# decadenza/SimpleStereo

Measured on AMD Instinct MI355X. Metric: disparity MPixels/s (H*W*nDisp per second), higher is better.
Workload: dtype f32

## Files before the change

simplestereo_amd/csrc/asw_exact_kernels.hip.h:

```cpp
#pragma once
#include "asw_shared.hip.h"
#include "lab_kernels.hip.h"
#include "glibc_math.hip.h"

namespace ssamd {

struct AswExactArgs {
    const PixRec *recL, *recR;
    const double *labL, *labR;
    const double *prox;
    u64 *keyL, *keyR;
    int16_t *disp;
    AswExactQueue q;
    AswExactQueue raw;
    double *ecost;
    u64 *costL, *costR;
    uint32_t *idxL, *idxR;
    uint32_t *wslotL, *wslotR;
    uint32_t *wpix;
    double *wtab;
    unsigned int wcap;
    int H, W, win, pad, minD, maxD, row0, rows;
    double gammaC;
};

__device__ __forceinline__ double exact_sqrt(double x)
{
#pragma clang fp contract(off)
    const double y0 = sqrt(x);
    if (!(y0 > 0.0) || !(y0 < 1.0e300)) return y0;
    const double e = fma(-y0, y0, x);
    return y0 + e / (2.0 * y0);
}

__global__ __launch_bounds__(256) void bgr2lab_f64_pair_kernel(const PixRec *__restrict__ recL, const PixRec *__restrict__ recR,
                                                               double *__restrict__ labL, double *__restrict__ labR, long long npix)
{
    SSAMD_LAB_TABLES_IN_LDS(T)
    long long q = (long long)blockIdx.x * blockDim.x + threadIdx.x;
    const long long stride = (long long)gridDim.x * blockDim.x;
    for (; q < 2 * npix; q += stride) {
        const bool right = q >= npix;
        const long long p = right ? q - npix : q;
        const uint32_t v = (right ? recR : recL)[p].bgrx;
        double L, a, b;
        bgr_to_lab_f64(v & 0xff, (v >> 8) & 0xff, (v >> 16) & 0xff, L, a, b, T);
        double *const o = (right ? labR : labL) + 3 * p;
        o[0] = L; o[1] = a; o[2] = b;
    }
}

__device__ __forceinline__ bool exact_overflowed(const AswExactArgs &A)
{
    return A.q.counter[0] > A.q.cap || (A.raw.entries && A.raw.counter[0] > A.raw.cap);
}

__global__ __launch_bounds__(256) void asw_exact_filter_kernel(const AswExactArgs A)
{
    const unsigned n = min(A.raw.counter[0], A.raw.cap);
    const unsigned nloop = (n + 255u) & ~255u;
    for (unsigned e0 = blockIdx.x * blockDim.x; e0 < nloop; e0 += gridDim.x * blockDim.x) {
        const unsigned e = e0 + threadIdx.x;
        unsigned s2 = 0;
        uint32_t pix = 0, rkey = 0xffffffffu;
        int d = 0;
        if (e < n) {
            const u64 ent = A.raw.entries[e];
            const uint32_t key = A.raw.ekeys[e];
            rkey = key;
            pix = (uint32_t)ent;
            d = (int)((ent >> 32) & 0xffff);
            const unsigned sides = (unsigned)(ent >> 48) & 3u;
            const uint32_t esc = 0xC0000000u - __float_as_uint(2.0f * A.q.sat_abs);
            if (sides & EXACT_SIDE_L) {
                const u64 g = A.keyL[pix];
                if ((int)(uint32_t)g != d && (uint32_t)(g >> 32) < esc && exact_near(key, (uint32_t)(g >> 32), A.q.tol, A.q.sat_abs, exact_zkey(A.win))) s2 |= EXACT_SIDE_L;
            }
            if ((sides & EXACT_SIDE_R) && A.keyR) {
                const u64 g = A.keyR[pix - (uint32_t)d];
                if ((uint32_t)g != pix % (uint32_t)A.W && (uint32_t)(g >> 32) < esc && exact_near(key, (uint32_t)(g >> 32), A.q.tol, A.q.sat_abs, exact_zkey(A.win))) s2 |= EXACT_SIDE_R;
            }
        }
        asw_exact_push_wave(A.q, s2 != 0, pix, d, s2, rkey);
    }
}

__global__ __launch_bounds__(256) void asw_exact_escalate_kernel(const AswExactArgs A)
{
    const AswExactQueue &Q = A.q;
    const uint32_t esc = 0xC0000000u - __float_as_uint(2.0f * Q.sat_abs);
    const long long n = (long long)A.rows * A.W;
    for (long long q = (long long)blockIdx.x * blockDim.x + threadIdx.x; q < n; q += (long long)gridDim.x * blockDim.x) {
        const int x = (int)(q % A.W);
        const u64 gl = A.keyL[q];
        if (gl != KEY_NONE && (uint32_t)(gl >> 32) >= esc) {
            const int dwin = (int)(uint32_t)gl, dhi = min(A.maxD, x);
            const int cnt = dhi - A.minD;
            if (cnt > 0) {
                unsigned slot = atomicAdd(Q.counter, (unsigned)cnt);
                for (int d = A.minD; d <= dhi; ++d)
                    if (d != dwin) {
                        if (slot < Q.cap) Q.entries[slot] = exact_entry((uint32_t)q, d, EXACT_SIDE_L);
                        ++slot;
                    }
                Q.flagL[q] = 1;
            }
        }
        if (A.keyR) {
            const u64 gr = A.keyR[q];
            if (gr != KEY_NONE && (uint32_t)(gr >> 32) >= esc) {
                const int xwin = (int)(uint32_t)gr;
                const int dhi = min(A.maxD, A.W - 1 - x), cnt = dhi - A.minD;
                if (cnt > 0) {
                    unsigned slot = atomicAdd(Q.counter, (unsigned)cnt);
                    for (int d = A.minD; d <= dhi; ++d)
                        if (x + d != xwin) {
                            if (slot < Q.cap) Q.entries[slot] = exact_entry((uint32_t)(q + d), d, EXACT_SIDE_R);
                            ++slot;
                        }
                    Q.flagR[q] = 1;
                }
            }
        }
    }
}

static constexpr int EXACT_ZSEG = 64, EXACT_ZWIN_MAX = 64;
__global__ __launch_bounds__(256) void asw_exact_zero_kernel(const AswExactArgs A)
{
    extern __shared__ __attribute__((aligned(16))) char zsmem[];
    const AswExactQueue &Q = A.q;
// ... 32 lines not shown
            }
            if (__syncthreads_or(tid < EXACT_ZSEG && s_state[tid] == 1) == 0) continue;
            if (win >= EXACT_ZWIN_MAX) {
                if (tid < EXACT_ZSEG && s_state[tid] == 1) s_state[tid] = 3;
            } else {
                const PixRec *const imgA = side ? A.recR : A.recL, *const imgB = side ? A.recL : A.recR;
                auto stage = [&](uint32_t *tile, const PixRec *img, int shift) {
                    for (int k0 = 0; k0 < win * TW; k0 += 8 * 256) {
                        uint32_t v[8];
#pragma unroll
                        for (int u = 0; u < 8; ++u) {
                            const int k = k0 + u * 256 + tid, i = k / TW, c = k - i * TW, ii = y - p + i, cc = x0 - p + c + shift;
                            v[u] = (k < win * TW && (unsigned)ii < (unsigned)H && (unsigned)cc < (unsigned)W) ? img[(size_t)ii * W + cc].bgrx : 0x80000000u;
                        }
#pragma unroll
                        for (int u = 0; u < 8; ++u) {
                            const int k = k0 + u * 256 + tid;
                            if (k < win * TW) tile[k] = v[u];
                        }
                    }
                };
                stage(tA, imgA, 0);
                for (;;) {
                    __syncthreads();
                    if (tid == 0) {
                        int cur = -1;
                        for (int k = 0; k < EXACT_ZSEG; ++k)
                            if (s_state[k] == 1) { cur = side ? s_idx[k] - (x0 + k) : s_idx[k]; break; }
                        s_cur = cur;
                    }
                    __syncthreads();
                    const int d = s_cur;
                    if (d < 0) break;
                    const int shift = side ? d : -d;
                    stage(tB, imgB, shift);
                    __syncthreads();
                    const int px = tid & (EXACT_ZSEG - 1), part = tid >> 6;
                    const bool mine = s_state[px] == 1 && (side ? s_idx[px] - (x0 + px) : s_idx[px]) == d;
                    bool nz = false;
                    if (mine) {
                        uint32_t acc = 0;
                        for (int i = part; i < win; i += 4) {
                            const uint32_t *const ra = tA + i * TW + px, *const rb = tB + i * TW + px;
#pragma unroll 8
                            for (int j = 0; j < win; ++j) {
                                const uint32_t a = ra[j], b = rb[j];
                                acc |= ((a | b) >> 31) ? 0u : (a ^ b);
                            }
                        }
                        nz = acc != 0u;
                    }
                    __syncthreads();
                    if (mine && part == 0) s_state[px] = 2;
                    __syncthreads();
                    if (mine && nz) s_state[px] = 3;
                }
            }
            __syncthreads();
            if (tid < EXACT_ZSEG && s_state[tid] == 3) {
                const int xq = x0 + tid, widx = s_idx[tid];
                const long long pq = (long long)yr * W + xq;
                if (side == 0) {
                    const int dhi = min(A.maxD, xq), cnt = dhi - A.minD;
                    if (cnt > 0) {
                        unsigned slot = atomicAdd(Q.counter, (unsigned)cnt);
                        for (int d = A.minD; d <= dhi; ++d)
                            if (d != widx) { if (slot < Q.cap) Q.entries[slot] = exact_entry((uint32_t)pq, d, EXACT_SIDE_L); ++slot; }
                        Q.flagL[pq] = 1;
                    }
                } else {
                    const int dhi = min(A.maxD, W - 1 - xq), cnt = dhi - A.minD;
                    if (cnt > 0) {
                        unsigned slot = atomicAdd(Q.counter, (unsigned)cnt);
                        for (int d = A.minD; d <= dhi; ++d)
                            if (xq + d != widx) { if (slot < Q.cap) Q.entries[slot] = exact_entry((uint32_t)(pq + d), d, EXACT_SIDE_R); ++slot; }
                        Q.flagR[pq] = 1;
                    }
                }
            }
        }
    }
}

__device__ __forceinline__ void exact_assign_wslot(const AswExactArgs &A, bool flagged, u64 mask, uint32_t pix, uint32_t side)
{
    if (mask == 0 || A.wcap == 0) return;
    const int leader = (int)__builtin_ctzll(mask);
    const unsigned lane = __builtin_amdgcn_mbcnt_hi(~0u, __builtin_amdgcn_mbcnt_lo(~0u, 0u));
    unsigned base = 0;
    if ((int)lane == leader) base = atomicAdd(A.q.counter + 6, (unsigned)__builtin_popcountll(mask));
    base = (unsigned)__builtin_amdgcn_readlane((int)base, leader);
    if (flagged) {
        const unsigned slot = base + (unsigned)__builtin_popcountll(mask & (((u64)1 << lane) - 1));
        (side ? A.wslotR : A.wslotL)[pix] = slot;
        if (slot < A.wcap) A.wpix[slot] = pix | (side << 31);
    }
}

__global__ __launch_bounds__(256) void asw_exact_winners_kernel(const AswExactArgs A)
{
    const AswExactQueue &Q = A.q;
    const long long n = (long long)A.rows * A.W;
    for (long long q0 = (long long)blockIdx.x * blockDim.x; q0 < n; q0 += (long long)gridDim.x * blockDim.x) {
        const long long q = q0 + threadIdx.x;
        const bool inb = q < n;
        const bool fl = inb && Q.flagL[q];
        if (fl) {
            A.costL[q] = ~0ull;
            A.idxL[q] = 0xffffffffu;
        }
        const int dwin = fl ? (A.keyL ? (int)(uint32_t)A.keyL[q] : (int)A.disp[q]) : 0;
        const u64 ml = __builtin_amdgcn_ballot_w64(fl);
        if (ml && fl && (int)__builtin_ctzll(ml) == (int)(threadIdx.x & 63)) atomicAdd(Q.counter + 1, (unsigned)__builtin_popcountll(ml));
        exact_assign_wslot(A, fl, ml, (uint32_t)q, 0u);
        asw_exact_push_wave(Q, fl, (uint32_t)q, dwin, EXACT_SIDE_L, fl && A.keyL ? (uint32_t)(A.keyL[q] >> 32) : 0xffffffffu);
        if (A.keyR) {
            const bool fr = inb && Q.flagR[q];
            int xl = 0, xr = 0;
            if (fr) {
                A.costR[q] = ~0ull;
                A.idxR[q] = 0xffffffffu;
                xr = (int)(q % A.W);
                xl = (int)(uint32_t)A.keyR[q];
            }
            const u64 mr = __builtin_amdgcn_ballot_w64(fr);
            if (mr && fr && (int)__builtin_ctzll(mr) == (int)(threadIdx.x & 63)) atomicAdd(Q.counter + 2, (unsigned)__builtin_popcountll(mr));
            exact_assign_wslot(A, fr, mr, (uint32_t)q, 1u);
            asw_exact_push_wave(Q, fr, (uint32_t)(q + (xl - xr)), xl - xr, EXACT_SIDE_R, fr ? (uint32_t)(A.keyR[q] >> 32) : 0xffffffffu);
        }
    }
}

__global__ __launch_bounds__(256) void asw_exact_wtab_kernel(const AswExactArgs A)
{
#pragma clang fp contract(off)
    __shared__ uint64_t s_exp[256];
    for (int k = threadIdx.x; k < 256; k += blockDim.x) s_exp[k] = gm_exp_tab[k];
    __syncthreads();
    if (exact_overflowed(A)) return;
    const unsigned n = min(A.q.counter[6], A.wcap);
    const int lane = threadIdx.x & 63, W = A.W, H = A.H, win = A.win, p = A.pad, win2 = win * win;
    for (unsigned slot = blockIdx.x * 4 + (threadIdx.x >> 6); slot < n; slot += gridDim.x * 4) {
        const uint32_t pw = A.wpix[slot], pix = pw & 0x7fffffffu;
        const double *const lab = (pw >> 31) ? A.labR : A.labL;
        const int yr = (int)(pix / (uint32_t)W), x = (int)(pix - (uint32_t)yr * (uint32_t)W), y = A.row0 + yr;
        const double *const c = lab + 3 * ((size_t)y * W + x);
        const double c0 = c[0], c1 = c[1], c2 = c[2];
        double *const out = A.wtab + (size_t)slot * win2;
        for (int t = lane; t < win2; t += 64) {
            const int i = t / win, j = t - i * win, ii = y - p + i, cc = x - p + j;
            double w = 0.0;
            if ((unsigned)ii < (unsigned)H && (unsigned)cc < (unsigned)W) {
                const double *const tp = lab + 3 * ((size_t)ii * W + cc);
                const double a0 = tp[0] - c0, a1 = tp[1] - c1, a2 = tp[2] - c2;
                w = A.prox[t] * glibc_exp_t(-exact_sqrt(a0 * a0 + a1 * a1 + a2 * a2) / A.gammaC, s_exp);
            }
            out[t] = w;
        }
    }
}

static constexpr int EXACT_WAVES = 4;
static constexpr int EXACT_CHUNK = 256;
__global__ __launch_bounds__(64 * EXACT_WAVES) void asw_exact_eval_kernel(const AswExactArgs A)
{
#pragma clang fp contract(off)
    __shared__ double s_w[EXACT_WAVES][EXACT_CHUNK], s_c[EXACT_WAVES][EXACT_CHUNK];
    __shared__ uint64_t s_exp[256];
    for (int k = threadIdx.x; k < 256; k += blockDim.x) s_exp[k] = gm_exp_tab[k];
    __syncthreads();
    if (exact_overflowed(A)) return;
    const int lane = threadIdx.x & 63, wv = threadIdx.x >> 6;
    double *const sw = s_w[wv], *const sc = s_c[wv];
    const unsigned n = min(A.q.counter[0], A.q.cap);
    const int W = A.W, H = A.H, win = A.win, p = A.pad;
    for (unsigned e = blockIdx.x * EXACT_WAVES + wv; e < n; e += gridDim.x * EXACT_WAVES) {
        const u64 ent = A.q.entries[e];
        const uint32_t pix = (uint32_t)ent;
        const int d = (int)((ent >> 32) & 0xffff);
        const unsigned sides = (unsigned)(ent >> 48) & 3u;
        const int yr = (int)(pix / (uint32_t)W), x = (int)(pix - (uint32_t)yr * (uint32_t)W);
        const int y = A.row0 + yr, xr = x - d;
        const double *const cl = A.labL + 3 * ((size_t)y * W + x), *const cr = A.labR + 3 * ((size_t)y * W + xr);
        const double cl0 = cl[0], cl1 = cl[1], cl2 = cl[2], cr0 = cr[0], cr1 = cr[1], cr2 = cr[2];
        const int jlo = max(0, p - xr), jhi = min(win, W + p - x), ncol = jhi - jlo;
        const int ilo = max(0, p - y), ihi = min(win, H + p - y);
        const int ntap = (ihi - ilo) * ncol;
        const uint32_t s1 = A.wcap && A.q.flagL && A.q.flagL[pix] ? A.wslotL[pix] : 0xffffffffu;
        const uint32_t s2 = A.wcap && A.q.flagR && A.q.flagR[pix - (uint32_t)d] ? A.wslotR[pix - (uint32_t)d] : 0xffffffffu;
        const double *const t1 = s1 < A.wcap ? A.wtab + (size_t)s1 * win * win : nullptr;
        const double *const t2 = s2 < A.wcap ? A.wtab + (size_t)s2 * win * win : nullptr;
        double acc = 0.0;
        bool all_zero = false;
        if ((unsigned)(ent >> 48) & EXACT_HINT_ZERO) {
            bool nz = false;
            for (int t = lane; t < ntap; t += 64) {
                const int q = t / ncol, i = ilo + q, j = jlo + (t - q * ncol);
                const int ii = y - p + i, jj = xr - p + j, kk = x - p + j;
                nz = nz || __builtin_amdgcn_sad_u8(A.recL[(size_t)ii * W + kk].bgrx, A.recR[(size_t)ii * W + jj].bgrx, 0u) != 0u;
            }
            all_zero = __builtin_amdgcn_ballot_w64(nz) == 0;
        }
        for (int t0 = 0; t0 < (all_zero ? 0 : ntap); t0 += EXACT_CHUNK) {
            const int nt = min(EXACT_CHUNK, ntap - t0);
            for (int t = lane; t < nt; t += 64) {
                const int q = (t0 + t) / ncol, i = ilo + q, j = jlo + (t0 + t - q * ncol);
                const int ii = y - p + i, jj = xr - p + j, kk = x - p + j;
                const double pr = A.prox[i * win + j];
                double w1, w2;
                if (t1) w1 = t1[i * win + j];
                else {
                    const double *const tl = A.labL + 3 * ((size_t)ii * W + kk);
                    const double a0 = tl[0] - cl0, a1 = tl[1] - cl1, a2 = tl[2] - cl2;
                    w1 = pr * glibc_exp_t(-exact_sqrt(a0 * a0 + a1 * a1 + a2 * a2) / A.gammaC, s_exp);
                }
                if (t2) w2 = t2[i * win + j];
                else {
                    const double *const tr = A.labR + 3 * ((size_t)ii * W + jj);
                    const double b0 = tr[0] - cr0, b1 = tr[1] - cr1, b2 = tr[2] - cr2;
                    w2 = pr * glibc_exp_t(-exact_sqrt(b0 * b0 + b1 * b1 + b2 * b2) / A.gammaC, s_exp);
                }
                const int tad = min(40, (int)__builtin_amdgcn_sad_u8(A.recL[(size_t)ii * W + kk].bgrx, A.recR[(size_t)ii * W + jj].bgrx, 0u));
                const double ww = w1 * w2;
                sw[t] = ww;
                sc[t] = ww * tad;
            }
            __builtin_amdgcn_wave_barrier();
            asm volatile("s_waitcnt lgkmcnt(0)" ::: "memory");
            if (lane < 2) {
                const double *const src = lane ? sw : sc;
                int t = 0;
                for (; t + 16 <= nt; t += 16) {
                    double v[16];
#pragma unroll
                    for (int u = 0; u < 16; ++u) v[u] = src[t + u];
#pragma unroll
                    for (int u = 0; u < 16; ++u) acc += v[u];
                }
                for (; t < nt; ++t) acc += src[t];
            }
            asm volatile("s_waitcnt lgkmcnt(0)" ::: "memory");
            __builtin_amdgcn_wave_barrier();
        }
        const double tot = __shfl(acc, 1);
        if (lane == 0) {
            const double c = all_zero ? 0.0 : acc / tot;
            A.ecost[e] = c;
            const u64 bits = (u64)__double_as_longlong(c);
            if (sides & EXACT_SIDE_L) atomicMin(A.costL + pix, bits);
            if (sides & EXACT_SIDE_R) atomicMin(A.costR + (pix - (uint32_t)d), bits);
        }
    }
}

__global__ __launch_bounds__(256) void asw_exact_resolve_kernel(const AswExactArgs A)
{
    if (exact_overflowed(A)) return;
    const unsigned n = A.q.counter[0];
    for (unsigned e = blockIdx.x * blockDim.x + threadIdx.x; e < n; e += gridDim.x * blockDim.x) {
        const u64 ent = A.q.entries[e];
        const uint32_t pix = (uint32_t)ent;
        const int d = (int)((ent >> 32) & 0xffff);
        const unsigned sides = (unsigned)(ent >> 48) & 3u;
        const u64 bits = (u64)__double_as_longlong(A.ecost[e]);
        if ((sides & EXACT_SIDE_L) && A.costL[pix] == bits) atomicMin(A.idxL + pix, (uint32_t)d);
        if ((sides & EXACT_SIDE_R) && A.costR[pix - (uint32_t)d] == bits) atomicMin(A.idxR + (pix - (uint32_t)d), pix % (uint32_t)A.W);
    }
}

__global__ __launch_bounds__(256) void asw_exact_patch_kernel(const AswExactArgs A)
{
    if (exact_overflowed(A)) return;
    const long long n = (long long)A.rows * A.W;
    for (long long q = (long long)blockIdx.x * blockDim.x + threadIdx.x; q < n; q += (long long)gridDim.x * blockDim.x) {
        if (A.q.flagL[q] && A.idxL[q] != 0xffffffffu) {
            if (A.keyL) A.keyL[q] = (A.keyL[q] & 0xffffffff00000000ull) | (u64)A.idxL[q];
            else A.disp[q] = (int16_t)A.idxL[q];
        }
        if (A.keyR && A.q.flagR[q] && A.idxR[q] != 0xffffffffu) A.keyR[q] = (A.keyR[q] & 0xffffffff00000000ull) | (u64)A.idxR[q];
    }
}

}
```

simplestereo_amd/csrc/host_asw_exact.h:

```cpp
namespace {
int get_prox64(Ctx &c, int win, double gammaP, hipStream_t s, const double **out);

int asw_exact_prepare(Ctx &c, int W, int rows, int win, int nD, double gammaC, bool consistent, bool direct, hipStream_t s,
                      AswExactQueue &q, AswExactQueue &raw, AswExactQueue &kernel_q)
{
    const size_t nout = (size_t)rows * W;
    if (nout >= ((size_t)1 << 32)) return fail(SSAMD_ELIMIT, "exact mode: more than 2^32 output pixels per call");
    const size_t all_cands = 2 * (nout * (size_t)nD + nout);
    size_t cap = std::min<size_t>(std::max<size_t>(4 * nout, std::min<size_t>(all_cands, (size_t)1 << 23)), (size_t)1 << 26);
    if (tune().exact_cap) cap = (size_t)tune().exact_cap;
    size_t rawcap = direct ? 0 : std::min<size_t>(std::max<size_t>(2 * nout, std::min<size_t>(all_cands, (size_t)1 << 23)), (size_t)1 << 26);
    if (!direct && tune().exact_cap) rawcap = std::max<size_t>(rawcap, cap);
    if (!direct && tune().exact_rawcap) rawcap = (size_t)tune().exact_rawcap;
    int rc;
    if ((rc = c.xqueue.reserve(cap * 8)) || (rc = c.xcost.reserve(cap * 8)) || (rc = c.xflags.reserve(64 + 4 * nout + (size_t)rows)) ||
        (rc = c.xslots.reserve(nout * 32)) || (rawcap && (rc = c.xraw.reserve(rawcap * 12))))
        return rc;
    c.xcap = (unsigned int)cap;
    c.xrawcap = (unsigned int)rawcap;
    HIP_TRY(hipMemsetAsync(c.xflags.ptr, 0, 64 + 4 * nout + (size_t)rows, s));
    q.entries = (u64 *)c.xqueue.ptr;
    q.ekeys = nullptr;
    q.counter = (unsigned int *)c.xflags.ptr;
    q.flagL = (unsigned char *)c.xflags.ptr + 64;
    q.flagR = consistent ? q.flagL + nout : nullptr;
    q.zeroL = q.flagL + 2 * nout;
    q.zeroR = consistent ? q.flagL + 3 * nout : nullptr;
    q.zrow = q.flagL + 4 * nout;
    q.W = (unsigned int)W;
    q.cap = (unsigned int)cap;
    q.tol = (uint32_t)std::min(1.0e6, (double)tune().exact_tol * std::max(1.0, 5.0 / gammaC) * std::max(1.0, win / 35.0));
    q.sat_abs = (float)(1.5 * 2.0 * 2.0 * ((double)win * win + 3.0) * 1.1102230246251565e-16 * 40.0);
    q.deep = 0xffffffffu;
    raw = AswExactQueue{};
    if (!direct) {
        raw = q;
        union { float f; uint32_t u; } sa; sa.f = q.sat_abs;
        raw.deep = 0xC0000000u - sa.u;
        raw.entries = (u64 *)c.xraw.ptr;
        raw.ekeys = (uint32_t *)((u64 *)c.xraw.ptr + rawcap);
        raw.counter = q.counter + 4;
        raw.flagL = raw.flagR = nullptr;
        raw.cap = (unsigned int)rawcap;
    }
    kernel_q = direct ? q : raw;
    return SSAMD_OK;
}

int asw_exact_pass(Ctx &c, const AswExactQueue &q, const AswExactQueue &raw, int H, int W, int row0, int rows, int win, int maxD, int minD, double gammaC, double gammaP,
                   bool consistent, bool direct, int16_t *d_disp, hipStream_t s)
{
    const int p = win / 2;
    const size_t nout = (size_t)rows * W, npix = (size_t)H * W;
    int rc;
    const double *d_prox = nullptr;
    if ((rc = get_prox64(c, win, gammaP, s, &d_prox))) return rc;
    if ((rc = c.xlabL.reserve(npix * 24)) || (rc = c.xlabR.reserve(npix * 24))) return rc;
    AswExactArgs x;
    x.recL = (const PixRec *)c.recL.ptr; x.recR = (const PixRec *)c.recR.ptr;
    x.labL = (const double *)c.xlabL.ptr; x.labR = (const double *)c.xlabR.ptr;
    x.prox = d_prox;
    x.keyL = direct ? nullptr : (u64 *)c.keyL.ptr; x.keyR = consistent ? (u64 *)c.keyR.ptr : nullptr;
    x.disp = d_disp;
    x.q = q;
    x.raw = raw;
    x.ecost = (double *)c.xcost.ptr;
    x.costL = (u64 *)c.xslots.ptr; x.costR = x.costL + nout;
    x.idxL = (uint32_t *)(x.costR + nout); x.idxR = x.idxL + nout;
    x.wslotL = x.idxR + nout; x.wslotR = x.wslotL + nout;
    {
        const size_t per = (size_t)win * win * 8;
        size_t wcap = std::min<size_t>(65536, ((size_t)64 << 20) / per);
        if (nout >= ((size_t)1 << 31)) wcap = 0;
        if (wcap && (rc = c.xwtab.reserve(wcap * 8 + wcap * per))) return rc;
        x.wcap = (unsigned int)wcap;
        x.wpix = (uint32_t *)c.xwtab.ptr;
        x.wtab = (double *)((char *)c.xwtab.ptr + wcap * 8);
    }
    x.H = H; x.W = W; x.win = win; x.pad = p; x.minD = minD; x.maxD = maxD; x.row0 = row0; x.rows = rows;
    x.gammaC = gammaC;
    Timed t(c, s, SSAMD_K_ASW_EXACT);
    {
        const int r0 = std::max(0, row0 - p), r1 = std::min(H, row0 + rows + p);
        const long long np2 = (long long)(r1 - r0) * W;
        const int blocks = (int)std::min<long long>((2 * np2 + 255) / 256, 256 * 8);
        hipLaunchKernelGGL(bgr2lab_f64_pair_kernel, dim3(blocks), dim3(256), 0, s, x.recL + (size_t)r0 * W, x.recR + (size_t)r0 * W,
                           (double *)c.xlabL.ptr + 3 * (size_t)r0 * W, (double *)c.xlabR.ptr + 3 * (size_t)r0 * W, np2);
    }
    const int pb = (int)std::min<long long>(((long long)nout + 255) / 256, 256 * 8);
    if (raw.entries) {
        hipLaunchKernelGGL(asw_exact_filter_kernel, dim3(256 * 8), dim3(256), 0, s, x);
        hipLaunchKernelGGL(asw_exact_escalate_kernel, dim3(pb), dim3(256), 0, s, x);
    }
    {
        const int zwin = std::min(win, EXACT_ZWIN_MAX - 1);
        const size_t zlds = (size_t)2 * zwin * (EXACT_ZSEG + 2 * (zwin / 2)) * 4;
        if ((rc = grant_dyn_lds(c, (const void *)asw_exact_zero_kernel, (int)zlds))) return rc;
        const long long segs = (long long)rows * ((W + EXACT_ZSEG - 1) / EXACT_ZSEG);
        hipLaunchKernelGGL(asw_exact_zero_kernel, dim3((unsigned)std::min<long long>(segs, 256 * 64)), dim3(256), zlds, s, x);
    }
    hipLaunchKernelGGL(asw_exact_winners_kernel, dim3(pb), dim3(256), 0, s, x);
    if (x.wcap) hipLaunchKernelGGL(asw_exact_wtab_kernel, dim3(256 * 4), dim3(256), 0, s, x);
    hipLaunchKernelGGL(asw_exact_eval_kernel, dim3((unsigned)(c.cus * 5)), dim3(64 * EXACT_WAVES), 0, s, x);
    hipLaunchKernelGGL(asw_exact_resolve_kernel, dim3(256 * 4), dim3(256), 0, s, x);
    hipLaunchKernelGGL(asw_exact_patch_kernel, dim3(pb), dim3(256), 0, s, x);
    HIP_TRY(hipGetLastError());
    ++c.exact_calls;
    return SSAMD_OK;
}

int asw_exact_counters(Ctx &c, unsigned int (&ctr)[5])
{
    std::fill(ctr, ctr + 5, 0u);
    if (!c.xflags.ptr || c.exact_calls == 0) return SSAMD_OK;
    HIP_TRY(hipDeviceSynchronize());
    HIP_TRY(hipMemcpy(ctr, c.xflags.ptr, sizeof(ctr), hipMemcpyDeviceToHost));
    return SSAMD_OK;
}
}
```

simplestereo_amd/csrc/host_debug.h:

```cpp
namespace {
extern "C" __global__ void debug_libm_kernel(int which, int n, const void *in, void *out)
{
    const int i = blockIdx.x * blockDim.x + threadIdx.x;
    if (i >= n) return;
    if (which == 0) reinterpret_cast<double *>(out)[i] = glibc_exp(reinterpret_cast<const double *>(in)[i]);
    else if (which == 1) reinterpret_cast<float *>(out)[i] = glibc_powf_pos(reinterpret_cast<const float *>(in)[i], (float)(1 / 3.0));
    else if (which == 2) reinterpret_cast<double *>(out)[i] = ssamd::exact_sqrt(reinterpret_cast<const double *>(in)[i]);
    else reinterpret_cast<double *>(out)[i] = reinterpret_cast<const double *>(in)[i] / 0.7 + reinterpret_cast<const double *>(in)[i] / 5.0;
}
}

extern "C" {
int ssamd_bgr2lab(const uint8_t *img, int height, int width, float *lab, int device)
{
    if (!img || !lab || height <= 0 || width <= 0) return fail(SSAMD_EINVAL, "bad argument");
    const size_t npix = (size_t)height * width;
    return host_route(device, {{&Ctx::imgL, img, npix * 3}}, {&Ctx::lab, lab, npix * 12}, [&](Ctx &c, hipStream_t s) {
        const int blocks = (int)std::min<size_t>((npix + 255) / 256, 256 * 8);
        hipLaunchKernelGGL(bgr2lab_f32_kernel, dim3(blocks), dim3(256), 0, s, (const uint8_t *)c.imgL.ptr, (float *)c.lab.ptr, (long long)npix);
        HIP_TRY(hipGetLastError());
        return SSAMD_OK;
    });
}

int ssamd_debug_exact_costs(const uint8_t *img1, const uint8_t *img2, int height, int width, int winSize, double gammaC, double gammaP,
                            int n, const int *yxd, double *costs, double *lab1, double *lab2)
{
    if (!img1 || !img2 || !yxd || !costs || n < 0) return fail(SSAMD_EINVAL, "NULL buffer");
    int rc = check_common(height, width, winSize, 0, 0, 0, height);
    if (rc) return rc;
    CtxLock c;
    if ((rc = get_ctx(-1, c))) return rc;
    const size_t npix = (size_t)height * width;
    hipStream_t s = c->stream;
    ScratchOrder order(*c, s);
    if ((rc = c->imgL.reserve(npix * 3)) || (rc = c->imgR.reserve(npix * 3)) || (rc = c->recL.reserve(npix * sizeof(PixRec))) ||
        (rc = c->recR.reserve(npix * sizeof(PixRec))) || (rc = c->xlabL.reserve(npix * 24)) || (rc = c->xlabR.reserve(npix * 24)) ||
        (rc = c->xqueue.reserve((size_t)std::max(n, 1) * 8)) || (rc = c->xcost.reserve((size_t)std::max(n, 1) * 8)) || (rc = c->xctr.reserve(64)))
        return rc;
    HIP_TRY(hipMemcpyAsync(c->imgL.ptr, img1, npix * 3, hipMemcpyHostToDevice, s));
    HIP_TRY(hipMemcpyAsync(c->imgR.ptr, img2, npix * 3, hipMemcpyHostToDevice, s));
    const int blocks = (int)std::min<long long>((2 * (long long)npix + 255) / 256, 256 * 8);
    hipLaunchKernelGGL(bgr2lab_records_pair_kernel, dim3(blocks), dim3(256), 0, s, (const uint8_t *)c->imgL.ptr, (const uint8_t *)c->imgR.ptr,
                       (PixRec *)c->recL.ptr, (PixRec *)c->recR.ptr, (long long)npix);
    hipLaunchKernelGGL(bgr2lab_f64_pair_kernel, dim3(blocks), dim3(256), 0, s, (const PixRec *)c->recL.ptr, (const PixRec *)c->recR.ptr,
                       (double *)c->xlabL.ptr, (double *)c->xlabR.ptr, (long long)npix);
    std::vector<u64> ent((size_t)n);
    for (int k = 0; k < n; ++k) {
        const int y = yxd[3 * k], x = yxd[3 * k + 1], d = yxd[3 * k + 2];
        if (y < 0 || y >= height || x < 0 || x >= width || d < 0 || x - d < 0) return fail(SSAMD_EINVAL, "candidate %d outside the image", k);
        ent[k] = (u64)((uint32_t)y * (uint32_t)width + (uint32_t)x) | ((u64)(uint32_t)d << 32);
    }
    const unsigned int ctr[16] = {(unsigned int)n};
    HIP_TRY(hipMemcpyAsync(c->xqueue.ptr, ent.data(), (size_t)n * 8, hipMemcpyHostToDevice, s));
    HIP_TRY(hipMemcpyAsync(c->xctr.ptr, ctr, sizeof(ctr), hipMemcpyHostToDevice, s));
    const double *d_prox = nullptr;
    if ((rc = get_prox64(*c, winSize, gammaP, s, &d_prox))) return rc;
    AswExactArgs x{};
    x.recL = (const PixRec *)c->recL.ptr; x.recR = (const PixRec *)c->recR.ptr;
    x.labL = (const double *)c->xlabL.ptr; x.labR = (const double *)c->xlabR.ptr;
    x.prox = d_prox; x.q.entries = (u64 *)c->xqueue.ptr; x.q.counter = (unsigned int *)c->xctr.ptr; x.q.cap = (unsigned int)std::max(n, 1);
    x.ecost = (double *)c->xcost.ptr;
    x.H = height; x.W = width; x.win = winSize; x.pad = winSize / 2; x.row0 = 0; x.rows = height; x.gammaC = gammaC;
    hipLaunchKernelGGL(asw_exact_eval_kernel, dim3(256), dim3(64 * EXACT_WAVES), 0, s, x);
    HIP_TRY(hipGetLastError());
    HIP_TRY(hipMemcpyAsync(costs, c->xcost.ptr, (size_t)n * 8, hipMemcpyDeviceToHost, s));
    if (lab1) HIP_TRY(hipMemcpyAsync(lab1, c->xlabL.ptr, npix * 24, hipMemcpyDeviceToHost, s));
    if (lab2) HIP_TRY(hipMemcpyAsync(lab2, c->xlabR.ptr, npix * 24, hipMemcpyDeviceToHost, s));
    HIP_TRY(hipStreamSynchronize(s));
    return SSAMD_OK;
}

int ssamd_debug_exact_queue(int which, long long max_n, unsigned long long *entries, unsigned int *keys, long long *n)
{
    if (!n || max_n < 0 || (max_n > 0 && !entries)) return fail(SSAMD_EINVAL, "bad argument");
    CtxLock c;
    int rc = get_ctx(-1, c);
    if (rc) return rc;
    *n = 0;
    unsigned int ctr[5];
    if ((rc = asw_exact_counters(*c, ctr))) return rc;
    const unsigned int cnt = which ? ctr[4] : ctr[0], cap = which ? c->xrawcap : c->xcap;
    *n = cnt;
    const size_t m = (size_t)std::min<long long>(std::min<unsigned int>(cnt, cap), max_n);
    if (m == 0) return SSAMD_OK;
    const void *src = which ? c->xraw.ptr : c->xqueue.ptr;
    if (!src) return SSAMD_OK;
    HIP_TRY(hipMemcpy(entries, src, m * 8, hipMemcpyDeviceToHost));
    if (which && keys) HIP_TRY(hipMemcpy(keys, (const char *)src + (size_t)c->xrawcap * 8, m * 4, hipMemcpyDeviceToHost));
    return SSAMD_OK;
}

int ssamd_debug_libm(int which, int n, const void *in, void *out)
{
    if (!in || !out || n < 0 || which < 0 || which > 3)
        return fail(SSAMD_EINVAL, "ssamd_debug_libm: which = 0 (exp, doubles), 1 (powf(x, 1/3), floats), 2 (sqrt, doubles), 3 (x / 0.7 + x / 5.0, doubles)");
    if (n == 0) return SSAMD_OK;
    const size_t bytes = (size_t)n * (which == 1 ? 4 : 8);
    return host_route(-1, {{&Ctx::lab, in, bytes, bytes}}, {&Ctx::lab, out, bytes}, [&](Ctx &c, hipStream_t s) {
        hipLaunchKernelGGL(debug_libm_kernel, dim3((n + 255) / 256), dim3(256), 0, s, which, n, (const void *)staged(c, &Ctx::lab, bytes),
                           (void *)staged(c, &Ctx::lab));
        HIP_TRY(hipGetLastError());
        return SSAMD_OK;
    });
}

int ssamd_debug_gsw_sqrt(int n, float *out)
{
    int what = 0;
    if (n < 0) { what = 1; n = -n; }
    if (!out || n <= 0 || n > GSW_TAB_SIZE) return fail(SSAMD_EINVAL, "bad argument");
    return host_route(-1, {}, {&Ctx::lab, out, (size_t)n * 4}, [&](Ctx &c, hipStream_t s) {
        hipLaunchKernelGGL(gsw_sqrt_probe_kernel, dim3((n + 255) / 256), dim3(256), 0, s, (float *)c.lab.ptr, n, what);
        HIP_TRY(hipGetLastError());
        return SSAMD_OK;
    });
}
}
```

simplestereo_amd/csrc/host_library.h:

```cpp
namespace {
int check_geometry_query(int width, int winSize, int maxDisparity, int minDisparity, const int *out, int *nD)
{
    if (!out) return fail(SSAMD_EINVAL, "out is NULL");
    int rc = check_common(1 << 14, width, winSize, minDisparity, maxDisparity, 0, 0);
    if (rc) return rc;
    *nD = maxDisparity - minDisparity + 1;
    return *nD < 1 ? fail(SSAMD_EINVAL, "empty disparity range") : SSAMD_OK;
}
}

extern "C" {
int ssamd_abi_version(void) { return SSAMD_ABI_VERSION; }
const char *ssamd_last_error(void) { return g_err.c_str(); }

int ssamd_device_count(void)
{
    int n = 0;
    if (hipGetDeviceCount(&n) != hipSuccess) return 0;
    return n;
}

const char *ssamd_kernel_name(int slot)
{
    static const char *names[SSAMD_K_COUNT] = {"asw pre-pass (asw_prepass_kernel: Lab records + TAD volume; or bgr2lab_records_pair_kernel, asw_tad_volume_kernel)", "asw aggregation kernel (asw_aggregate_pipe / _wave / asw_aggregate_kernel)",
                                               "asw finalize (wta_decode / lr_check_fill)",
                                               "gsw_aggregate_kernel", "gsw finalize (lr_check_fill)", "remap_bgr_kernel / ftp_reference_kernel", "reproject_kernel / ftp_cloud_kernel",
                                               "asw_alt_fill_kernel", "asw fp64 tie-break pass (bgr2lab_f64_pair + asw_exact_winners / _eval / _resolve / _patch kernels)",
                                               "iir_unwrap_kernel", "ftp_phase_kernel", "np_unwrap_row_kernel / np_unwrap_col_kernel"};
    return (slot >= 0 && slot < SSAMD_K_COUNT) ? names[slot] : "";
}

int ssamd_set_option(const char *name, const char *value)
{
    if (!name) return fail(SSAMD_EINVAL, "option name is NULL");
    std::lock_guard<std::mutex> lk(g_tune_mutex);
    if (value) {
        if (!tuning_assign(g_tuning, name, value)) return fail(SSAMD_EINVAL, "unknown option %s", name);
    } else {
        const auto it = g_tuning_env.find(name);
        if (!tuning_assign(g_tuning, name, it == g_tuning_env.end() ? nullptr : it->second.c_str()))
            return fail(SSAMD_EINVAL, "unknown option %s", name);
    }
    if (std::string(name) == "SSAMD_AUTOTUNE")
        g_autotune.store(g_tuning.autotune_env != -2 ? g_tuning.autotune_env : -1);
    g_tune_version.fetch_add(1, std::memory_order_release);
    return SSAMD_OK;
}

int ssamd_counter(int device, const char *name, long long *value)
{
    if (!name || !value) return fail(SSAMD_EINVAL, "name / value is NULL");
    CtxLock c;
    int rc = get_ctx(device, c);
    if (rc) return rc;
    const std::string n(name);
    if (n == "evol_fallbacks") *value = c->evol_fallbacks;
    else if (n == "evol_bytes") *value = (long long)c->evol.cap;
    else if (n == "tail_splits") *value = c->tail_splits;
    else if (n == "exact_calls") *value = c->exact_calls;
    else if (n == "pipe_persist_launches") *value = c->persist_launches;
    else if (n == "gsw_plain_calls") *value = c->gsw_plain_calls;
    else if (n == "pipe_persist_items") {
        unsigned long long done = 0;
        if (c->pq.ptr) {
            HIP_TRY(hipDeviceSynchronize());
            HIP_TRY(hipMemcpy(&done, (const unsigned int *)c->pq.ptr + ASW_PQ_QUEUES * ASW_PQ_LINE, sizeof(done), hipMemcpyDeviceToHost));
        }
        *value = (long long)done;
    }
    else if (n == "exact_entries" || n == "exact_flagged_left" || n == "exact_flagged_right" || n == "exact_overflow" || n == "exact_raw_entries") {
        unsigned int ctr[5];
        if ((rc = asw_exact_counters(*c, ctr))) return rc;
        *value = n == "exact_entries" ? ctr[0] : n == "exact_flagged_left" ? ctr[1] : n == "exact_flagged_right" ? ctr[2] :
                 n == "exact_raw_entries" ? ctr[4] : ((ctr[0] > c->xcap || (c->xrawcap && ctr[4] > c->xrawcap)) ? 1 : 0);
    }
    else return fail(SSAMD_EINVAL, "unknown counter %s", name);
    return SSAMD_OK;
}

int ssamd_autotune(int on)
{
    return g_autotune.exchange(on > 0 ? 1 : (on < 0 ? -1 : 0));
}

int ssamd_asw_geometry(int width, int rows, int winSize, int maxDisparity, int minDisparity, int *out)
{
    int nD, rc = check_geometry_query(width, winSize, maxDisparity, minDisparity, out, &nD);
    if (rc) return rc;
    const Tuning &t = tune();
    const PlanOptions po{t, false};
    AswGeom g;
    if ((rc = asw_choose_geometry(g, po, width, rows, winSize, nD))) return rc;
    out[0] = g.Tx; out[1] = g.Dc; out[2] = g.nchunks; out[3] = g.threads; out[4] = g.lds_bytes;
    out[5] = (width + g.Tx - 1) / g.Tx; out[6] = rows; out[7] = g.nchunks;
    AswWaveGeom wg;
    if (g.wave_rx && asw_wave_layout(wg, po, winSize, nD, g.wave_rx, t.wave_unroll != 0)) {
        out[0] = wg.Txw * wg.waves; out[1] = wg.Dc; out[2] = 1; out[3] = 64 * wg.waves; out[4] = wg.wave_lds * wg.waves;
        out[5] = (width + out[0] - 1) / out[0]; out[7] = 1;
    }
    return SSAMD_OK;
}

int ssamd_asw_kernel_form(int width, int rows, int winSize, int maxDisparity, int minDisparity, int *out)
{
    int nD, rc = check_geometry_query(width, winSize, maxDisparity, minDisparity, out, &nD);
    if (rc) return rc;
    const Tuning &t = tune();
    AswGeom g;
    if ((rc = asw_choose_geometry(g, PlanOptions{t, false}, width, rows, winSize, nD))) return rc;
    out[0] = g.pipe; out[1] = g.Rx; out[2] = g.JC >= winSize ? 0 : g.JC; out[3] = g.pipe ? g.dephase : 0;
    out[4] = g.wave_rx & 15;
    if (g.wave_rx) { out[0] = 0; out[1] = g.wave_rx & 15; out[2] = 0; out[3] = 0; }
    return SSAMD_OK;
}

int ssamd_gsw_geometry(int width, int rows, int winSize, int maxDisparity, int minDisparity, int *out)
{
    int nD, rc = check_geometry_query(width, winSize, maxDisparity, minDisparity, out, &nD);
    if (rc) return rc;
    GswGeom g;
    if ((rc = gsw_choose_geometry(g, tune(), width, rows, winSize, nD))) return rc;
    out[0] = g.Tx; out[1] = g.Dc; out[2] = g.nchunks; out[3] = g.threads * g.Hy; out[4] = g.lds_bytes;
    out[5] = (width + g.Tx - 1) / g.Tx; out[6] = (rows + g.Ty * g.Hy - 1) / (g.Ty * g.Hy); out[7] = g.nchunks; out[8] = g.Ty * g.Hy;
    return SSAMD_OK;
}

int ssamd_profile_enable(int on)
{
    for (auto &c : g_ctx) {
        std::lock_guard<std::mutex> lk(c.mu);
        c.prof.on = on != 0;
    }
    return SSAMD_OK;
}

int ssamd_profile_reset(void)
{
    DeviceGuard guard;
    for (auto &c : g_ctx) {
        std::lock_guard<std::mutex> lk(c.mu);
        if (c.dev < 0) continue;
        (void)hipSetDevice(c.dev);
        c.prof.drain();
        std::fill(c.prof.ms, c.prof.ms + SSAMD_K_COUNT, 0.0);
        std::fill(c.prof.n, c.prof.n + SSAMD_K_COUNT, 0LL);
    }
    return SSAMD_OK;
}

int ssamd_profile_read(double *ms, long long *launches)
{
    DeviceGuard guard;
    for (int k = 0; k < SSAMD_K_COUNT; ++k) { if (ms) ms[k] = 0; if (launches) launches[k] = 0; }
    for (auto &c : g_ctx) {
        std::lock_guard<std::mutex> lk(c.mu);
        if (c.dev < 0) continue;
// ... 8 lines not shown
```

simplestereo_amd/csrc/ssamd_options.h:

```cpp
#pragma once

#define SSAMD_OPTIONS(X) \
    X("SSAMD_ASW_GEOM", asw_geom, std::string, "", v, !x.empty())    \
    X("SSAMD_GSW_GEOM", gsw_geom, std::string, "", v, false) \
    X("SSAMD_GSW_PLAIN", gsw_plain, int, 0, atoi(v) != 0 ? 1 : 0, false)    \
    X("SSAMD_ASW_PIPE", asw_pipe, int, -1, atoi(v), x >= 0)    \
    X("SSAMD_ASW_DEPHASE", asw_dephase, int, -1, atoi(v), x >= 0)    \
    X("SSAMD_ASW_EVOL", asw_evol, int, 1, atoi(v), x != 1)    \
    X("SSAMD_ASW_WAVE", asw_wave, int, -1, atoi(v) != 0 ? 1 : 0, x >= 0)    \
    X("SSAMD_ASW_WAVE_RX", wave_rx, int, 0, atoi(v), x != 0)    \
    X("SSAMD_ASW_WAVE_WG", wave_wg, int, 0, std::max(1, std::min(4, atoi(v))), x != 0)    \
    X("SSAMD_ASW_WAVE_UNROLL", wave_unroll, int, 1, atoi(v), false)    \
    X("SSAMD_ASW_WAVE_MERGE", wave_merge, int, 1, atoi(v), x == 0)    \
    X("SSAMD_ASW_STATIC", asw_static, int, 1, atoi(v), x != 1)    \
    X("SSAMD_ASW_EVOL_MAX_MB", evol_max_mb, int, 0, std::max(0, atoi(v)), x != 0)    \
    X("SSAMD_ASW_WAVE_RD", wave_rd, int, 0, atoi(v), x != 0)    \
    X("SSAMD_ASW_NO_E2", no_e2, bool, false, true, x) \
    X("SSAMD_ASW_XOR_ONLY", xor_only, bool, false, true, x) \
    X("SSAMD_MULTI_ALLOW_REPEAT", multi_allow_repeat, bool, false, true, false) \
    X("SSAMD_ALT_QUEUE_CAP", alt_queue_cap, int, 0, std::max(1, atoi(v)), false)    \
    X("SSAMD_AUTOTUNE", autotune_env, int, -2, atoi(v) > 0 ? 1 : (atoi(v) < 0 ? -1 : 0), false)    \
    X("SSAMD_ASW_EVOL_FAIL", evol_fail, int, 0, atoi(v), false)    \
    X("SSAMD_ASW_TAIL", asw_tail, int, -1, atoi(v), false)    \
    X("SSAMD_ASW_PERSIST", asw_persist, int, -1, atoi(v), x > 0)    \
    X("SSAMD_ASW_PREPASS_FUSE", prepass_fuse, int, 1, atoi(v), false)    \
    X("SSAMD_EXACT_TOL", exact_tol, int, 128, std::max(0, atoi(v)), false)    \
    X("SSAMD_EXACT_CAP", exact_cap, int, 0, std::max(1, atoi(v)), false)    \
    X("SSAMD_EXACT_RAWCAP", exact_rawcap, int, 0, std::max(1, atoi(v)), false)    \
    X("SSAMD_UNWRAP_ROWS", unwrap_rows, int, 0, std::max(0, std::min(UNWRAP_MAX_ROWS, atoi(v))), false)

struct Tuning {
#define X(NAME, MEMBER, TYPE, UNSET, PARSE, FORCES) TYPE MEMBER = UNSET;
    SSAMD_OPTIONS(X)
#undef X
};

bool tuning_assign(Tuning &t, const std::string &name, const char *v)
{
#define X(NAME, MEMBER, TYPE, UNSET, PARSE, FORCES) \
    if (name == NAME) { if (v) t.MEMBER = PARSE; else t.MEMBER = UNSET; return true; }
    SSAMD_OPTIONS(X)
#undef X
    return false;
}

const char *const kTuningNames[] = {
#define X(NAME, MEMBER, TYPE, UNSET, PARSE, FORCES) NAME,
    SSAMD_OPTIONS(X)
#undef X
};

bool asw_geometry_forced(const Tuning &t)
{
#define X(NAME, MEMBER, TYPE, UNSET, PARSE, FORCES) { const TYPE &x = t.MEMBER; (void)x; if (FORCES) return true; }
    SSAMD_OPTIONS(X)
#undef X
    return false;
}
```

Baseline: 10690.

## Mark needed rows and right centres to skip Lab work and reuse weight tables

Adds a mark kernel that flags which image rows the exact-recheck entries touch and which right-image centres need precomputed weight tables. The f64 Lab conversion then runs only on marked rows, and the wtab kernel builds tables for those extra right centres so the eval kernel can take a fast path that reads both tables and uses SAD on packed bytes. It also changes the wtab kernel to one block per slot and replaces the tap index division with a float reciprocal. The cost is an extra kernel launch with atomics and more flag memory. The risk is correctness if the row mask or slot bookkeeping misses a case.

```diff
diff --git a/simplestereo_amd/csrc/asw_exact_kernels.hip.h b/simplestereo_amd/csrc/asw_exact_kernels.hip.h
--- a/simplestereo_amd/csrc/asw_exact_kernels.hip.h
+++ b/simplestereo_amd/csrc/asw_exact_kernels.hip.h
@@ -20,6 +20,8 @@
     uint32_t *wpix;
     double *wtab;
     unsigned int wcap;
+    unsigned char *markR;
+    unsigned char *rowmask;
     int H, W, win, pad, minD, maxD, row0, rows;
     double gammaC;
 };
@@ -34,19 +36,24 @@
 }
 
 __global__ __launch_bounds__(256) void bgr2lab_f64_pair_kernel(const PixRec *__restrict__ recL, const PixRec *__restrict__ recR,
-                                                               double *__restrict__ labL, double *__restrict__ labR, long long npix)
+                                                               double *__restrict__ labL, double *__restrict__ labR, int nrows, int W,
+                                                               const unsigned char *__restrict__ rowmask)
 {
     SSAMD_LAB_TABLES_IN_LDS(T)
-    long long q = (long long)blockIdx.x * blockDim.x + threadIdx.x;
-    const long long stride = (long long)gridDim.x * blockDim.x;
-    for (; q < 2 * npix; q += stride) {
-        const bool right = q >= npix;
-        const long long p = right ? q - npix : q;
-        const uint32_t v = (right ? recR : recL)[p].bgrx;
-        double L, a, b;
-        bgr_to_lab_f64(v & 0xff, (v >> 8) & 0xff, (v >> 16) & 0xff, L, a, b, T);
-        double *const o = (right ? labR : labL) + 3 * p;
-        o[0] = L; o[1] = a; o[2] = b;
+    const int segs = (W + 255) / 256;
+    for (long long u = blockIdx.x; u < (long long)nrows * segs; u += gridDim.x) {
+        const int r = (int)(u / segs), x = (int)(u - (long long)r * segs) * 256 + (int)threadIdx.x;
+        if (rowmask && !rowmask[r]) continue;
+        if (x < W) {
+            const size_t p = (size_t)r * W + x;
+            const uint32_t vl = recL[p].bgrx, vr = recR[p].bgrx;
+            double L0, a0, b0, L1, a1, b1;
+            bgr_to_lab_f64(vl & 0xff, (vl >> 8) & 0xff, (vl >> 16) & 0xff, L0, a0, b0, T);
+            bgr_to_lab_f64(vr & 0xff, (vr >> 8) & 0xff, (vr >> 16) & 0xff, L1, a1, b1, T);
+            double *const ol = labL + 3 * p, *const orr = labR + 3 * p;
+            ol[0] = L0; ol[1] = a0; ol[2] = b0;
+            orr[0] = L1; orr[1] = a1; orr[2] = b1;
+        }
     }
 }
 
@@ -245,9 +252,9 @@
     }
 }
 
-__device__ __forceinline__ void exact_assign_wslot(const AswExactArgs &A, bool flagged, u64 mask, uint32_t pix, uint32_t side)
-{
-    if (mask == 0 || A.wcap == 0) return;
+__device__ __forceinline__ uint32_t exact_assign_wslot(const AswExactArgs &A, bool flagged, u64 mask, uint32_t pix, uint32_t side)
+{
+    if (mask == 0 || A.wcap == 0) return 0xffffffffu;
     const int leader = (int)__builtin_ctzll(mask);
     const unsigned lane = __builtin_amdgcn_mbcnt_hi(~0u, __builtin_amdgcn_mbcnt_lo(~0u, 0u));
     unsigned base = 0;
@@ -257,7 +264,9 @@
         const unsigned slot = base + (unsigned)__builtin_popcountll(mask & (((u64)1 << lane) - 1));
         (side ? A.wslotR : A.wslotL)[pix] = slot;
         if (slot < A.wcap) A.wpix[slot] = pix | (side << 31);
-    }
+        return slot;
+    }
+    return 0xffffffffu;
 }
 
 __global__ __launch_bounds__(256) void asw_exact_winners_kernel(const AswExactArgs A)
@@ -294,6 +303,42 @@
     }
 }
 
+__global__ __launch_bounds__(256) void asw_exact_mark_kernel(const AswExactArgs A)
+{
+    if (exact_overflowed(A)) return;
+    const unsigned n = min(A.q.counter[0], A.q.cap);
+    const unsigned nloop = (n + 255u) & ~255u;
+    const unsigned lane = threadIdx.x & 63u;
+    for (unsigned e0 = blockIdx.x * blockDim.x; e0 < nloop; e0 += gridDim.x * blockDim.x) {
+        const unsigned e = e0 + threadIdx.x;
+        bool first = false, own = false;
+        uint32_t r = 0;
+        if (e < n) {
+            const u64 ent = A.q.entries[e];
+            const uint32_t pix = (uint32_t)ent;
+            if (A.markR) {
+                r = pix - (uint32_t)((ent >> 32) & 0xffff);
+                unsigned char *const a = A.markR + r;
+                const unsigned sh = 8u * (unsigned)((uintptr_t)a & 3u);
+                first = ((atomicOr(reinterpret_cast<unsigned int *>((uintptr_t)a & ~(uintptr_t)3), 1u << sh) >> sh) & 0xffu) == 0u;
+                own = first && A.q.flagR && A.q.flagR[r];
+            }
+            if (first || !A.markR) {
+                const int k0 = (int)(pix / (uint32_t)A.W);
+                const int klo = max(k0, A.pad - A.row0), khi = min(k0 + 2 * A.pad, A.H - 1 - A.row0 + A.pad);
+                for (int k = klo; k <= khi; ++k) A.rowmask[k] = 1;
+            }
+        }
+        if (!A.markR) continue;
+        const bool want = first && !own;
+        const uint32_t slot = exact_assign_wslot(A, want, __builtin_amdgcn_ballot_w64(want), r, 1u);
+        const bool served = A.wcap && first && (own ? A.wslotR[r] : slot) < A.wcap;
+        const u64 mf = __builtin_amdgcn_ballot_w64(first), ms = __builtin_amdgcn_ballot_w64(served);
+        if (mf && (int)__builtin_ctzll(mf) == (int)lane) atomicAdd(A.q.counter + 8, (unsigned)__builtin_popcountll(mf));
+        if (ms && (int)__builtin_ctzll(ms) == (int)lane) atomicAdd(A.q.counter + 9, (unsigned)__builtin_popcountll(ms));
+    }
+}
+
 __global__ __launch_bounds__(256) void asw_exact_wtab_kernel(const AswExactArgs A)
 {
 #pragma clang fp contract(off)
@@ -302,15 +347,15 @@
     __syncthreads();
     if (exact_overflowed(A)) return;
     const unsigned n = min(A.q.counter[6], A.wcap);
-    const int lane = threadIdx.x & 63, W = A.W, H = A.H, win = A.win, p = A.pad, win2 = win * win;
-    for (unsigned slot = blockIdx.x * 4 + (threadIdx.x >> 6); slot < n; slot += gridDim.x * 4) {
+    const int W = A.W, H = A.H, win = A.win, p = A.pad, win2 = win * win;
+    for (unsigned slot = blockIdx.x; slot < n; slot += gridDim.x) {
         const uint32_t pw = A.wpix[slot], pix = pw & 0x7fffffffu;
         const double *const lab = (pw >> 31) ? A.labR : A.labL;
         const int yr = (int)(pix / (uint32_t)W), x = (int)(pix - (uint32_t)yr * (uint32_t)W), y = A.row0 + yr;
         const double *const c = lab + 3 * ((size_t)y * W + x);
         const double c0 = c[0], c1 = c[1], c2 = c[2];
         double *const out = A.wtab + (size_t)slot * win2;
-        for (int t = lane; t < win2; t += 64) {
+        for (int t = threadIdx.x; t < win2; t += 256) {
             const int i = t / win, j = t - i * win, ii = y - p + i, cc = x - p + j;
             double w = 0.0;
             if ((unsigned)ii < (unsigned)H && (unsigned)cc < (unsigned)W) {
@@ -349,8 +394,10 @@
         const int jlo = max(0, p - xr), jhi = min(win, W + p - x), ncol = jhi - jlo;
         const int ilo = max(0, p - y), ihi = min(win, H + p - y);
         const int ntap = (ihi - ilo) * ncol;
+        const float rcol = 1.0f / (float)ncol;
+        const uint32_t rpix = pix - (uint32_t)d;
         const uint32_t s1 = A.wcap && A.q.flagL && A.q.flagL[pix] ? A.wslotL[pix] : 0xffffffffu;
-        const uint32_t s2 = A.wcap && A.q.flagR && A.q.flagR[pix - (uint32_t)d] ? A.wslotR[pix - (uint32_t)d] : 0xffffffffu;
+        const uint32_t s2 = A.wcap && ((A.q.flagR && A.q.flagR[rpix]) || (A.markR && A.markR[rpix])) ? A.wslotR[rpix] : 0xffffffffu;
         const double *const t1 = s1 < A.wcap ? A.wtab + (size_t)s1 * win * win : nullptr;
         const double *const t2 = s2 < A.wcap ? A.wtab + (size_t)s2 * win * win : nullptr;
         double acc = 0.0;
@@ -366,8 +413,40 @@
         }
         for (int t0 = 0; t0 < (all_zero ? 0 : ntap); t0 += EXACT_CHUNK) {
             const int nt = min(EXACT_CHUNK, ntap - t0);
-            for (int t = lane; t < nt; t += 64) {
-                const int q = (t0 + t) / ncol, i = ilo + q, j = jlo + (t0 + t - q * ncol);
+            auto tap_ij = [&](int tt, int &i, int &j) {
+                int q = (int)((float)tt * rcol), rj = tt - q * ncol;
+                if (rj < 0) { --q; rj += ncol; }
+                else if (rj >= ncol) { ++q; rj -= ncol; }
+                i = ilo + q; j = jlo + rj;
+            };
+            if (t1 && t2) {
+                constexpr int NU = EXACT_CHUNK / 64;
+                double w1[NU], w2[NU];
+                uint32_t bl[NU], br[NU];
+#pragma unroll
+                for (int u = 0; u < NU; ++u) {
+                    int i, j;
+                    tap_ij(t0 + min(lane + 64 * u, nt - 1), i, j);
+                    const size_t row = (size_t)(y - p + i) * W;
+                    w1[u] = t1[i * win + j];
+                    w2[u] = t2[i * win + j];
+                    bl[u] = A.recL[row + (x - p + j)].bgrx;
+                    br[u] = A.recR[row + (xr - p + j)].bgrx;
+                }
+#pragma unroll
+                for (int u = 0; u < NU; ++u) {
+                    const int t = lane + 64 * u;
+                    const int tad = min(40, (int)__builtin_amdgcn_sad_u8(bl[u], br[u], 0u));
+                    const double ww = w1[u] * w2[u];
+                    if (t < nt) {
+                        sw[t] = ww;
+                        sc[t] = ww * tad;
+                    }
+                }
+            }
+            else for (int t = lane; t < nt; t += 64) {
+                int i, j;
+                tap_ij(t0 + t, i, j);
                 const int ii = y - p + i, jj = xr - p + j, kk = x - p + j;
                 const double pr = A.prox[i * win + j];
                 double w1, w2;
diff --git a/simplestereo_amd/csrc/host_asw_exact.h b/simplestereo_amd/csrc/host_asw_exact.h
--- a/simplestereo_amd/csrc/host_asw_exact.h
+++ b/simplestereo_amd/csrc/host_asw_exact.h
@@ -1,5 +1,12 @@
 namespace {
 int get_prox64(Ctx &c, int win, double gammaP, hipStream_t s, const double **out);
+
+size_t exact_rowmask_offset(size_t nout, int rows) { return 64 + 4 * nout + (size_t)rows; }
+size_t exact_own_mark_offset(size_t nout, int rows, int win) { return (exact_rowmask_offset(nout, rows) + (size_t)rows + 2 * (size_t)(win / 2) + 3) & ~(size_t)3; }
+size_t exact_flag_bytes(size_t nout, int rows, int win, bool consistent)
+{
+    return exact_own_mark_offset(nout, rows, win) + (consistent ? ((nout + 3) & ~(size_t)3) : 0);
+}
 
 int asw_exact_prepare(Ctx &c, int W, int rows, int win, int nD, double gammaC, bool consistent, bool direct, hipStream_t s,
                       AswExactQueue &q, AswExactQueue &raw, AswExactQueue &kernel_q)
@@ -13,12 +20,13 @@
     if (!direct && tune().exact_cap) rawcap = std::max<size_t>(rawcap, cap);
     if (!direct && tune().exact_rawcap) rawcap = (size_t)tune().exact_rawcap;
     int rc;
-    if ((rc = c.xqueue.reserve(cap * 8)) || (rc = c.xcost.reserve(cap * 8)) || (rc = c.xflags.reserve(64 + 4 * nout + (size_t)rows)) ||
+    const size_t fbytes = exact_flag_bytes(nout, rows, win, consistent);
+    if ((rc = c.xqueue.reserve(cap * 8)) || (rc = c.xcost.reserve(cap * 8)) || (rc = c.xflags.reserve(fbytes)) ||
         (rc = c.xslots.reserve(nout * 32)) || (rawcap && (rc = c.xraw.reserve(rawcap * 12))))
         return rc;
     c.xcap = (unsigned int)cap;
     c.xrawcap = (unsigned int)rawcap;
-    HIP_TRY(hipMemsetAsync(c.xflags.ptr, 0, 64 + 4 * nout + (size_t)rows, s));
+    HIP_TRY(hipMemsetAsync(c.xflags.ptr, 0, fbytes, s));
     q.entries = (u64 *)c.xqueue.ptr;
     q.ekeys = nullptr;
     q.counter = (unsigned int *)c.xflags.ptr;
@@ -72,6 +80,7 @@
         const size_t per = (size_t)win * win * 8;
         size_t wcap = std::min<size_t>(65536, ((size_t)64 << 20) / per);
         if (nout >= ((size_t)1 << 31)) wcap = 0;
+        if (tune().exact_wcap) wcap = std::min<size_t>(wcap, (size_t)tune().exact_wcap);
         if (wcap && (rc = c.xwtab.reserve(wcap * 8 + wcap * per))) return rc;
         x.wcap = (unsigned int)wcap;
         x.wpix = (uint32_t *)c.xwtab.ptr;
@@ -79,14 +88,9 @@
     }
     x.H = H; x.W = W; x.win = win; x.pad = p; x.minD = minD; x.maxD = maxD; x.row0 = row0; x.rows = rows;
     x.gammaC = gammaC;
+    x.rowmask = (unsigned char *)c.xflags.ptr + exact_rowmask_offset(nout, rows);
+    x.markR = !tune().exact_rtab || !x.wcap ? nullptr : consistent ? (unsigned char *)c.xflags.ptr + exact_own_mark_offset(nout, rows, win) : q.flagL + nout;
     Timed t(c, s, SSAMD_K_ASW_EXACT);
-    {
-        const int r0 = std::max(0, row0 - p), r1 = std::min(H, row0 + rows + p);
-        const long long np2 = (long long)(r1 - r0) * W;
-        const int blocks = (int)std::min<long long>((2 * np2 + 255) / 256, 256 * 8);
-        hipLaunchKernelGGL(bgr2lab_f64_pair_kernel, dim3(blocks), dim3(256), 0, s, x.recL + (size_t)r0 * W, x.recR + (size_t)r0 * W,
-                           (double *)c.xlabL.ptr + 3 * (size_t)r0 * W, (double *)c.xlabR.ptr + 3 * (size_t)r0 * W, np2);
-    }
     const int pb = (int)std::min<long long>(((long long)nout + 255) / 256, 256 * 8);
     if (raw.entries) {
         hipLaunchKernelGGL(asw_exact_filter_kernel, dim3(256 * 8), dim3(256), 0, s, x);
@@ -100,7 +104,15 @@
         hipLaunchKernelGGL(asw_exact_zero_kernel, dim3((unsigned)std::min<long long>(segs, 256 * 64)), dim3(256), zlds, s, x);
     }
     hipLaunchKernelGGL(asw_exact_winners_kernel, dim3(pb), dim3(256), 0, s, x);
-    if (x.wcap) hipLaunchKernelGGL(asw_exact_wtab_kernel, dim3(256 * 4), dim3(256), 0, s, x);
+    hipLaunchKernelGGL(asw_exact_mark_kernel, dim3(256), dim3(256), 0, s, x);
+    {
+        const int r0 = std::max(0, row0 - p), r1 = std::min(H, row0 + rows + p);
+        const long long units = (long long)(r1 - r0) * ((W + 255) / 256);
+        hipLaunchKernelGGL(bgr2lab_f64_pair_kernel, dim3((unsigned)std::min<long long>(units, 256 * 8)), dim3(256), 0, s, x.recL + (size_t)r0 * W,
+                           x.recR + (size_t)r0 * W, (double *)c.xlabL.ptr + 3 * (size_t)r0 * W, (double *)c.xlabR.ptr + 3 * (size_t)r0 * W, r1 - r0, W,
+                           (const unsigned char *)x.rowmask + (r0 - row0 + p));
+    }
+    if (x.wcap) hipLaunchKernelGGL(asw_exact_wtab_kernel, dim3(256 * 8), dim3(256), 0, s, x);
     hipLaunchKernelGGL(asw_exact_eval_kernel, dim3((unsigned)(c.cus * 5)), dim3(64 * EXACT_WAVES), 0, s, x);
     hipLaunchKernelGGL(asw_exact_resolve_kernel, dim3(256 * 4), dim3(256), 0, s, x);
     hipLaunchKernelGGL(asw_exact_patch_kernel, dim3(pb), dim3(256), 0, s, x);
@@ -109,9 +121,9 @@
     return SSAMD_OK;
 }
 
-int asw_exact_counters(Ctx &c, unsigned int (&ctr)[5])
+int asw_exact_counters(Ctx &c, unsigned int (&ctr)[10])
 {
-    std::fill(ctr, ctr + 5, 0u);
+    std::fill(ctr, ctr + 10, 0u);
     if (!c.xflags.ptr || c.exact_calls == 0) return SSAMD_OK;
     HIP_TRY(hipDeviceSynchronize());
     HIP_TRY(hipMemcpy(ctr, c.xflags.ptr, sizeof(ctr), hipMemcpyDeviceToHost));
diff --git a/simplestereo_amd/csrc/host_debug.h b/simplestereo_amd/csrc/host_debug.h
--- a/simplestereo_amd/csrc/host_debug.h
+++ b/simplestereo_amd/csrc/host_debug.h
@@ -44,7 +44,7 @@
     hipLaunchKernelGGL(bgr2lab_records_pair_kernel, dim3(blocks), dim3(256), 0, s, (const uint8_t *)c->imgL.ptr, (const uint8_t *)c->imgR.ptr,
                        (PixRec *)c->recL.ptr, (PixRec *)c->recR.ptr, (long long)npix);
     hipLaunchKernelGGL(bgr2lab_f64_pair_kernel, dim3(blocks), dim3(256), 0, s, (const PixRec *)c->recL.ptr, (const PixRec *)c->recR.ptr,
-                       (double *)c->xlabL.ptr, (double *)c->xlabR.ptr, (long long)npix);
+                       (double *)c->xlabL.ptr, (double *)c->xlabR.ptr, height, width, (const unsigned char *)nullptr);
     std::vector<u64> ent((size_t)n);
     for (int k = 0; k < n; ++k) {
         const int y = yxd[3 * k], x = yxd[3 * k + 1], d = yxd[3 * k + 2];
@@ -78,16 +78,16 @@
     int rc = get_ctx(-1, c);
     if (rc) return rc;
     *n = 0;
-    unsigned int ctr[5];
+    unsigned int ctr[10];
     if ((rc = asw_exact_counters(*c, ctr))) return rc;
-    const unsigned int cnt = which ? ctr[4] : ctr[0], cap = which ? c->xrawcap : c->xcap;
+    const unsigned int cnt = which == 1 ? ctr[4] : ctr[0], cap = which == 1 ? c->xrawcap : c->xcap;
     *n = cnt;
     const size_t m = (size_t)std::min<long long>(std::min<unsigned int>(cnt, cap), max_n);
     if (m == 0) return SSAMD_OK;
-    const void *src = which ? c->xraw.ptr : c->xqueue.ptr;
+    const void *src = which == 1 ? c->xraw.ptr : which == 2 ? c->xcost.ptr : c->xqueue.ptr;
     if (!src) return SSAMD_OK;
     HIP_TRY(hipMemcpy(entries, src, m * 8, hipMemcpyDeviceToHost));
-    if (which && keys) HIP_TRY(hipMemcpy(keys, (const char *)src + (size_t)c->xrawcap * 8, m * 4, hipMemcpyDeviceToHost));
+    if (which == 1 && keys) HIP_TRY(hipMemcpy(keys, (const char *)src + (size_t)c->xrawcap * 8, m * 4, hipMemcpyDeviceToHost));
     return SSAMD_OK;
 }
 
diff --git a/simplestereo_amd/csrc/host_library.h b/simplestereo_amd/csrc/host_library.h
--- a/simplestereo_amd/csrc/host_library.h
+++ b/simplestereo_amd/csrc/host_library.h
@@ -68,10 +68,11 @@
         }
         *value = (long long)done;
     }
-    else if (n == "exact_entries" || n == "exact_flagged_left" || n == "exact_flagged_right" || n == "exact_overflow" || n == "exact_raw_entries") {
-        unsigned int ctr[5];
+    else if (n == "exact_entries" || n == "exact_flagged_left" || n == "exact_flagged_right" || n == "exact_overflow" || n == "exact_raw_entries" ||
+             n == "exact_right_centres" || n == "exact_right_tables") {
+        unsigned int ctr[10];
         if ((rc = asw_exact_counters(*c, ctr))) return rc;
-        *value = n == "exact_entries" ? ctr[0] : n == "exact_flagged_left" ? ctr[1] : n == "exact_flagged_right" ? ctr[2] :
+        *value = n == "exact_right_centres" ? ctr[8] : n == "exact_right_tables" ? ctr[9] : n == "exact_entries" ? ctr[0] : n == "exact_flagged_left" ? ctr[1] : n == "exact_flagged_right" ? ctr[2] :
                  n == "exact_raw_entries" ? ctr[4] : ((ctr[0] > c->xcap || (c->xrawcap && ctr[4] > c->xrawcap)) ? 1 : 0);
     }
     else return fail(SSAMD_EINVAL, "unknown counter %s", name);
diff --git a/simplestereo_amd/csrc/ssamd_options.h b/simplestereo_amd/csrc/ssamd_options.h
--- a/simplestereo_amd/csrc/ssamd_options.h
+++ b/simplestereo_amd/csrc/ssamd_options.h
@@ -27,6 +27,8 @@
     X("SSAMD_EXACT_TOL", exact_tol, int, 128, std::max(0, atoi(v)), false)    \
     X("SSAMD_EXACT_CAP", exact_cap, int, 0, std::max(1, atoi(v)), false)    \
     X("SSAMD_EXACT_RAWCAP", exact_rawcap, int, 0, std::max(1, atoi(v)), false)    \
+    X("SSAMD_EXACT_RTAB", exact_rtab, int, 1, atoi(v) != 0 ? 1 : 0, false)    \
+    X("SSAMD_EXACT_WCAP", exact_wcap, int, 0, std::max(1, atoi(v)), false)    \
     X("SSAMD_UNWRAP_ROWS", unwrap_rows, int, 0, std::max(0, std::min(UNWRAP_MAX_ROWS, atoi(v))), false)
 
 struct Tuning {
```

After: 10710 (median of 6 runs). About the same (+0.2%).
